# feos-org/feos-torch

Measured on AMD Instinct MI355X. Metric: pc_saft_pure_vapor_pressure_solves_per_sec, higher is better.
Workload: dtype f64 (fp32 pre-solve, fp64 finish)

## Files before the change

### feos_torch_amd/_lib.py

```python
import ctypes
import os

_HERE = os.path.dirname(os.path.abspath(__file__))
LIB_PATH = os.environ.get("PCS_HIP_LIB") or os.path.join(_HERE, "libpcsaft_hip.so")

_lib = None

_vp = ctypes.c_void_p
_i64 = ctypes.c_int64
_int = ctypes.c_int

SIGNATURES = {
    "pcs_abi_version": (_int, []),
    "pcs_last_error": (ctypes.c_char_p, []),
    "pcs_workspace_bytes": (_i64, [_i64]),
    "pcs_pure_vle": (_int, [_vp, _vp, _i64, _vp, _vp, _vp, _vp, _vp, _vp, _vp]),
    "pcs_pure_vapor_pressure": (_int, [_vp, _vp, _i64, _vp, _vp, _vp, _vp, _vp]),
    "pcs_compact_workspace_bytes": (_i64, [_i64]),
    "pcs_compact_plan": (_int, [_vp, _i64, _vp, _vp]),
    "pcs_compact_rows": (_int, [_vp, _i64, _vp, _vp, _int, _vp, _vp, _vp]),
    "pcs_expand_rows": (_int, [_vp, _i64, _vp, _vp, _vp, _int, _int, _int, _vp, _vp]),
    "pcs_pure_vle_fast": (_int, [_vp, _vp, _i64, _vp, _vp, _vp, _vp, _vp, _vp, _vp]),
    "pcs_pure_row_order": (_int, [_vp, _vp, _i64, _vp, _vp]),
    "pcs_pure_vle_fast_ordered": (_int, [_vp, _vp, _i64, _vp, _vp, _vp, _vp, _vp, _vp, _vp, _vp]),
    "pcs_pure_vle_fp64": (_int, [_vp, _vp, _i64, _vp, _vp, _vp, _vp, _vp, _vp, _vp]),
    "pcs_pure_vle_retry": (_int, [_vp, _vp, _i64, _vp, _vp, _vp, _vp, _vp, _vp, _vp]),
    "pcs_pure_liquid_density": (_int, [_vp, _vp, _vp, _i64, _vp, _vp, _vp, _vp]),
    "pcs_pure_derivatives": (_int, [_vp, _vp, _vp, _i64, _vp, _vp, _vp, _vp]),
    "pcs_pure_start_probe": (_int, [_vp, _vp, _i64, _vp, _vp]),
    "pcs_pure_jacobian": (_int, [_int, _vp, _vp, _vp, _vp, _i64, _vp, _vp]),
    "pcs_pure_jacobian_vjp": (_int, [_int, _vp, _vp, _vp, _vp, _vp, _i64, _vp, _vp, _vp, _vp]),
    "pcs_pure_critical_point": (_int, [_vp, _vp, _i64, _vp, _vp, _vp, _vp, _vp, _vp]),
    "pcs_pure_critical_point_vjp": (_int, [_vp, _vp, _vp, _i64, _vp, _vp, _vp, _vp, _vp]),
    "pcs_pure_boiling_temperature": (_int, [_vp, _vp, _vp, _i64, _vp, _vp, _vp, _vp, _vp]),
    "pcs_pure_enthalpy_of_vaporization": (_int, [_vp, _vp, _i64, _vp, _vp, _vp, _vp]),
    "pcs_pure_enthalpy_of_vaporization_vjp": (_int, [_vp, _vp, _vp, _i64, _vp, _vp, _vp, _vp]),
    "pcs_mix_workspace_bytes": (_i64, [_i64]),
    "pcs_mix_bubble_dew": (_int, [_int, _vp, _vp, _vp, _vp, _vp, _i64, _vp, _vp, _vp, _vp, _vp, _vp]),
    "pcs_mix_bubble_dew_temperature": (_int, [_int, _vp, _vp, _vp, _vp, _vp, _i64, _vp, _vp, _vp, _vp, _vp, _vp]),
    "pcs_mix_density": (_int, [_int, _vp, _vp, _vp, _vp, _vp, _i64, _vp, _vp, _vp, _vp, _vp, _vp]),
    "pcs_mix_henry": (_int, [_int, _vp, _vp, _vp, _i64, _vp, _vp, _vp, _vp, _vp, _vp]),
    "pcs_mix_jacobian": (_int, [_int, _vp, _vp, _vp, _vp, _i64, _vp, _vp, _vp]),
    "pcs_mix_point_jacobian": (_int, [_int, _vp, _vp, _vp, _vp, _i64, _vp, _vp, _vp, _vp]),
    "pcs_gc_table_doubles": (_i64, [_int]),
    "pcs_gc_bubble_dew": (_int, [_int, _vp, _int, _vp, _vp, _vp, _vp, _vp, _i64, _vp, _vp, _vp, _vp, _vp, _vp, _vp]),
    "pcs_gc_bubble_dew_temperature": (_int, [_int, _vp, _int, _vp, _vp, _vp, _vp, _vp, _i64, _vp, _vp, _vp, _vp, _vp, _vp]),
    "pcs_gc_density": (_int, [_int, _vp, _int, _vp, _vp, _vp, _vp, _vp, _i64, _vp, _vp, _vp, _vp, _vp, _vp]),
    "pcs_gc_pure_vle": (_int, [_int, _vp, _int, _vp, _vp, _vp, _i64, _vp, _vp, _vp, _vp, _vp, _vp, _vp]),
    "pcs_gc_derivatives": (_int, [_vp, _int, _vp, _vp, _vp, _vp, _i64, _vp, _vp, _vp, _vp, _vp]),
    "pcs_gc_jacobian": (_int, [_int, _vp, _int, _vp, _vp, _vp, _vp, _i64, _vp, _vp, _vp, _vp]),
    "pcs_gc_segment_gradient": (_int, [_int, _vp, _int, _vp, _vp, _vp, _vp, _i64, _vp, _vp, _vp, _vp]),
    "pcs_gc_point_jacobian": (_int, [_int, _vp, _int, _vp, _vp, _vp, _vp, _i64, _vp, _vp, _vp, _vp, _vp]),
    "pcs_gc_point_segment_gradient": (_int, [_int, _vp, _int, _vp, _vp, _vp, _vp, _i64, _vp, _vp, _vp, _vp, _vp]),
    "pcs_pure_derivatives_vjp": (_int, [_vp, _vp, _vp, _i64, _vp, _vp, _vp, _vp, _vp, _vp, _vp]),
    "pcs_mix_derivatives_vjp": (_int, [_vp, _vp, _vp, _vp, _i64, _vp, _vp, _vp, _vp, _vp, _vp, _vp]),
    "pcs_gc_derivatives_vjp": (_int, [_vp, _int, _vp, _vp, _vp, _vp, _i64, _vp, _vp, _vp, _vp, _vp, _vp, _vp, _vp, _vp]),
    "pcs_mixn_derivatives": (_int, [_vp, _vp, _vp, _int, _i64, _vp, _vp, _vp, _vp, _vp]),
    "pcs_mixn_derivatives_vjp": (_int, [_vp, _vp, _vp, _int, _i64, _vp, _vp, _vp, _vp, _vp, _vp]),
    "pcs_mix_derivatives": (_int, [_vp, _vp, _vp, _vp, _i64, _vp, _vp, _vp, _vp, _vp]),
    "pcs_mix_stability": (_int, [_vp, _vp, _vp, _vp, _i64, _vp, _vp, _vp, _vp]),
    "pcs_gc_stability": (_int, [_vp, _int, _vp, _vp, _vp, _vp, _i64, _vp, _vp, _vp, _vp, _vp]),
}


class PcsError(RuntimeError):
    pass


def lib():
    global _lib
    if _lib is None:
        if not os.path.exists(LIB_PATH):
            raise PcsError(
                f"{LIB_PATH} not found: build it with `python -c 'import __graft_entry__ as g; g.build()'` "
                "(hipcc --offload-arch=gfx950). There is no CPU fallback."
            )
        L = ctypes.CDLL(LIB_PATH)
        for name, (res, args) in SIGNATURES.items():
            fn = getattr(L, name)
            fn.restype = res
            fn.argtypes = args
        _lib = L
    return _lib


def check(rc, what):
    if rc != 0:
        msg = lib().pcs_last_error().decode("utf-8", "replace")
        raise PcsError(f"{what} failed (rc={rc}): {msg}")


def ptr(t):
    if t is None:
        return None
    return ctypes.c_void_p(t.data_ptr())


def current_stream_ptr(device):
    import torch

    return ctypes.c_void_p(torch.cuda.current_stream(device).cuda_stream)
```

### feos_torch_amd/csrc/pure_f32.hpp

```cpp
#pragma once
#include "pure_model.hpp"

namespace pcs {

constexpr float PCS_F32_TAYLOR_MAX = 1e-3f;
constexpr float PCS_F32_PREDICT_TOL_L = 5e-6f;
constexpr float PCS_F32_PREDICT_TOL_V = 5e-5f;
constexpr float PCS_F32_PREDICT_CMAX = 1e3f;
constexpr int PCS_F32_DENSE_LEVELS = 3;
constexpr float PCS_F32_LEAN_MAX = 0.5f;
constexpr float PCS_F32_SECANT_MIN = 3e-4f;
constexpr float PCS_F32_LIQ_TOL = 1e-1f;

struct F2 {
    float v, d1, d2;
};
PCS_DEV F2 f2(float v, float d1, float d2) { F2 r; r.v = v; r.d1 = d1; r.d2 = d2; return r; }
PCS_DEV F2 operator+(F2 a, F2 b) { return f2(a.v + b.v, a.d1 + b.d1, a.d2 + b.d2); }
PCS_DEV F2 operator-(F2 a, F2 b) { return f2(a.v - b.v, a.d1 - b.d1, a.d2 - b.d2); }
PCS_DEV F2 operator+(F2 a, float b) { return f2(a.v + b, a.d1, a.d2); }
PCS_DEV F2 operator-(float b, F2 a) { return f2(b - a.v, -a.d1, -a.d2); }
PCS_DEV F2 operator*(F2 a, float b) { return f2(a.v * b, a.d1 * b, a.d2 * b); }
PCS_DEV F2 operator*(F2 a, F2 b) {
    return f2(a.v * b.v, fmaf(a.d1, b.v, a.v * b.d1), fmaf(a.d2, b.v, fmaf(2.0f * a.d1, b.d1, a.v * b.d2)));
// ... 339 lines not shown
static_assert(start_close(START.SB[0], start_horner(B0, (double)PCS_F32_START_ETA)) && start_close(START.SB[1], start_horner(B1, (double)PCS_F32_START_ETA)) &&
              start_close(START.SB[2], start_horner(B2, (double)PCS_F32_START_ETA)), "eta-moments of B0..B2 against their Horner evaluation");
static_assert(start_close(start_log(6.0), 2.0 * start_log(2.0) + start_log(1.5)) && start_close(start_log(0.001) + start_log(1000.0), 0.0) &&
              start_close(start_log(2.718281828459045), 1.0), "compile-time logarithm");

PCS_DEV float start_rho_f32(const PureCoefF& c) { return PCS_F32_START_ETA / c.ceta; }

PCS_DEV EvalF pure_eval_start_f32(const PureCoefF& c) {
    constexpr StartConst K = START;
    const float rho = start_rho_f32(c);
    const float F = c.m * (float)K.HS.v - c.mm1 * (float)K.LG.v;
    const float Ft = c.m * (float)K.HS.t - c.mm1 * (float)K.LG.t;
    const float Ftt = c.m * (float)K.HS.tt - c.mm1 * (float)K.LG.tt;
    const float m1 = c.m1, m2 = c.m2;
    const float I1 = fmaf(m1, fmaf(m2, (float)K.SA[2].v, (float)K.SA[1].v), (float)K.SA[0].v);
    const float I1t = fmaf(m1, fmaf(m2, (float)K.SA[2].t, (float)K.SA[1].t), (float)K.SA[0].t);
    const float I1tt = fmaf(m1, fmaf(m2, (float)K.SA[2].tt, (float)K.SA[1].tt), (float)K.SA[0].tt);
    const float I2 = fmaf(m1, fmaf(m2, (float)K.SB[2].v, (float)K.SB[1].v), (float)K.SB[0].v);
    const float I2t = fmaf(m1, fmaf(m2, (float)K.SB[2].t, (float)K.SB[1].t), (float)K.SB[0].t);
    const float I2tt = fmaf(m1, fmaf(m2, (float)K.SB[2].tt, (float)K.SB[1].tt), (float)K.SB[0].tt);
    const float D = 1.0f + c.m * (float)K.A.v - c.mm1 * (float)K.B.v;
    const float Dt = c.m * (float)K.A.t - c.mm1 * (float)K.B.t;
    const float Dtt = c.m * (float)K.A.tt - c.mm1 * (float)K.B.tt;
    const float C = __builtin_amdgcn_rcpf(D), Csq = C * C;
    const float Ct = -Dt * Csq;
    const float Ctt = (2.0f * Dt * Dt * C - Dtt) * Csq;
    const float G = c.kd1 * I1 + c.kd2 * (C * I2);
    const float Gt = c.kd1 * I1t + c.kd2 * (Ct * I2 + C * I2t);
    const float Gtt = c.kd1 * I1tt + c.kd2 * (Ctt * I2 + 2.0f * Ct * I2t + C * I2tt);
    float a = rho * (F + rho * G);
    float at = rho * (F + Ft + rho * (2.0f * G + Gt));
    float att = rho * (2.0f * Ft + Ftt + rho * (2.0f * G + 4.0f * Gt + Gtt));
    if (c.polar || c.assoc) {
        if (c.polar) {
            float j1v = c.j1[0], j1t = 0.0f, j1tt = 0.0f, j2v = c.j2[0], j2t = 0.0f, j2tt = 0.0f;
#pragma unroll
            for (int i = 1; i < 5; i++) {
                j1v = fmaf(c.j1[i], K.pw.v[i], j1v);
                j1t = fmaf(c.j1[i], K.pw.t[i], j1t);
                if (i > 1) j1tt = fmaf(c.j1[i], K.pw.tt[i], j1tt);
            }
#pragma unroll
            for (int i = 1; i < 4; i++) {
                j2v = fmaf(c.j2[i], K.pw.v[i], j2v);
                j2t = fmaf(c.j2[i], K.pw.t[i], j2t);
                if (i > 1) j2tt = fmaf(c.j2[i], K.pw.tt[i], j2tt);
            }
            const F2 J1 = f2(j1v, j1t, j1tt);
            const F2 N = f2(j2v, j2t, j2tt) * rho;
            const F2 Q = (J1 * J1) * recipf(J1 - f2(N.v, N.d1 + N.v, N.d2 + 2.0f * N.d1));
            const float k = (rho * rho) * c.qm;
            a = fmaf(k, Q.v, a);
            at = fmaf(k, Q.d1 + 2.0f * Q.v, at);
            att = fmaf(k, Q.d2 + 4.0f * Q.d1 + 2.0f * Q.v, att);
        }
        if (c.assoc) {
            const float rd = rho * c.da;
            const float S = rd * (float)K.H.v, St = rd * (float)K.H.t, Stt = rd * (float)K.H.tt;
            float xa, xb;
            assoc_sites_f32(c, S, xa, xb);
            const float q = c.na * (f_log(xa) - 0.5f * xa + 0.5f) + c.nb * (f_log(xb) - 0.5f * xb + 0.5f);
            const float nn = c.na * c.nb;
            const float q1 = -nn * xa * xb;
            const float al = c.nb * xa * xa, be = c.na * xb * xb;
            const float rden = __builtin_amdgcn_rcpf(1.0f - al * be * S * S);
            const float xa1 = al * (be * S * xa - xb) * rden, xb1 = be * (al * S * xb - xa) * rden;
            const float q2 = -nn * (xa1 * xb + xa * xb1);
            a = fmaf(rho, q, a);
            at = fmaf(rho, q + q1 * St, at);
            att = fmaf(rho, q1 * (2.0f * St + Stt) + q2 * St * St, att);
        }
    }
    const float ir = c.ceta * (1.0f / PCS_F32_START_ETA);
    EvalF e;
    e.a = a;
    e.p = rho - a + at;
    e.dp = fmaf(att, ir, 1.0f);
    e.mu = at * ir;
    return e;
}

PCS_DEV bool finitef(float x) { return (__float_as_uint(x) & 0x7f800000u) != 0x7f800000u; }

struct LiquidRootF {
    float rl;
    bool ok, done, dense;
    int first;
};
template <bool AT_START>
PCS_DEV void liquid_root_step(const PureCoefF& f, float p_spec, float tol, float tol_dense, int it, const EvalF& e, LiquidRootF& s) {
    const float res = e.p - p_spec;
    const float eta = AT_START ? PCS_F32_START_ETA : s.rl * f.ceta;
    const int rung = AT_START ? 0 : eta < 0.575f ? 0 : eta < 0.655f ? 1 : eta < 0.735f ? 2 : PCS_F32_DENSE_LEVELS;
    if (it == s.first && rung < PCS_F32_DENSE_LEVELS && finitef(e.p) && !(res > 0.0f)) {
        s.dense = true;
        s.first = it + 1;
        float rn = (0.58f + 0.08f * (float)rung) / f.ceta;
        if (AT_START && e.dp > 0.0f) {
            const float r1 = s.rl - res * __builtin_amdgcn_rcpf(e.dp);
            const float eta1 = r1 * f.ceta;
            if (finitef(r1) && eta1 > PCS_F32_START_ETA && eta1 <= 0.74f) rn = r1;
        }
        s.rl = rn;
    } else if (!finitef(e.p) || !(e.dp > 0.0f) || (it == s.first && !(res > 0.0f))) {
        s.ok = false;
        s.done = true;
    } else {
        const float u = AT_START ? (float)START.u : __builtin_amdgcn_rcpf(1.0f - s.rl * f.ceta);
        float den = s.dense ? e.dp : e.dp - 4.0f * res * f.ceta * u;
        float step = res * __builtin_amdgcn_rcpf(den);
        if (!(den > 0.0f)) step = 2.0f * s.rl;
        float rn = s.rl - step;
        if (!(rn > 0.0f)) { s.ok = false; s.done = true; }
        else { s.done = fabsf(step) <= (s.dense ? tol_dense : tol) * s.rl; s.rl = rn; }
    }
}
PCS_DEV bool liquid_root_f32(const PureCoefF& f, float p_spec, float tol, float tol_dense, int cap, float& rl,
                             int& n_eval) {
    LiquidRootF s;
    s.ok = finitef(f.da) && finitef(f.kd2) && finitef(f.ceta) && f.ceta > 0.0f && finitef(p_spec);
    s.rl = start_rho_f32(f);
    s.done = !s.ok;
    s.dense = false;
    s.first = 0;
    if (cap > 0) {
        if (!s.done) {
            liquid_root_step<true>(f, p_spec, tol, tol_dense, 0, pure_eval_start_f32(f), s);
            n_eval++;
        }
        if (__ballot(!s.done) != 0ull) {
#pragma unroll 1
            for (int it = 1; it < cap; it++) {
                if (!s.done) {
                    liquid_root_step<false>(f, p_spec, tol, tol_dense, it, pure_eval_f32(f, s.rl), s);
                    n_eval++;
                }
                if (__ballot(!s.done) == 0ull) break;
            }
        }
    }
    rl = s.rl;
    return s.ok && s.done;
}

struct PreState {
    float rl, rv;
    EvalF l;
    float dpv;
    float sl_prev, sv_prev;
    float pv, dv_taken;
    float ev;
    float sec_prev, d_prev;
    bool lean_v;
    int it, n_liq, code;
    bool ok, done;
};

PCS_DEV void presolve_begin(const PureCoefF& f, PreState& s) {
    s.n_liq = 0; s.it = 0; s.code = 0;
    s.dpv = 1.0f; s.sl_prev = 1.0f; s.sv_prev = 1.0f;
    s.pv = 0.0f; s.dv_taken = 0.0f; s.ev = 0.0f; s.sec_prev = 0.0f; s.d_prev = 0.0f; s.lean_v = false;
    bool ok = liquid_root_f32(f, 0.0f, PCS_F32_LIQ_TOL, 1e-2f, 12, s.rl, s.n_liq);
    const float rl = s.rl;
    s.l = pure_eval_f32(f, rl);
    float rv = rl * f_exp(s.l.mu);
    {
        float B = (4.0f * f.m - 2.5f * f.mm1) * f.ceta + f.kd1 * f.ai[0] + f.kd2 * f.bi[0];
        if (f.polar) B += f.qm * f.j1[0];
        if (f.assoc) B -= f.na * f.nb * f.da;
        const float Lg = f_log(rv);
        float r = rv;
#pragma unroll
        for (int k = 0; k < 3; k++) {
            float den = fmaxf(1.0f + 2.0f * B * r, 0.3f);
            float fr = f_log(r) + 2.0f * B * r - Lg;
            r = r * fmaxf(1.0f - fr * __builtin_amdgcn_rcpf(den), 0.2f);
        }
        if (finitef(r) && r > 0.0f) rv = r;
    }
    s.code = !ok ? 1 : !finitef(rv) ? 6 : !(s.l.dp > 0.0f) ? 7 : !(rv < 0.5f * rl) ? 8 : !(rv > 1e-30f) ? 9 : 0;
    ok = ok && finitef(rv) && (s.l.dp > 0.0f) && (rv < 0.5f * rl) && (rv > 1e-30f);
    s.rv = rv;
    s.ok = ok;
    s.done = !ok;
}

PCS_DEV bool carry_slope(float p0, float p1, float drho, float s, float mu, float& dp, float& err, float& sec_prev, float& d_prev) {
    if (!(s * dp >= PCS_F32_SECANT_MIN * (1.0f + fabsf(mu)))) {
        d_prev = 0.0f;
        return true;
    }
    const float sec = (p1 - p0) * __builtin_amdgcn_rcpf(drho);
    const bool three = d_prev != 0.0f && fabsf(drho) <= 0.5f * fabsf(d_prev);
    const float cand = three ? fmaf(sec - sec_prev, drho * __builtin_amdgcn_rcpf(d_prev + drho), sec) : fmaf(2.0f, sec, -dp);
    if (!finitef(cand) || !(cand > 0.0f)) return false;
    const float rel = fabsf(cand * __builtin_amdgcn_rcpf(dp) - 1.0f);
    err = three ? 0.5f * rel * __builtin_amdgcn_sqrtf(err) : 0.25f * rel * rel;
    dp = cand;
    sec_prev = sec;
    d_prev = drho;
    return true;
}

PCS_DEV void presolve_coupled(const PureCoefF& f, PreState& s, int it_end) {
    float rl = s.rl, rv = s.rv;
    EvalF l = s.l;
    bool ok = s.ok, done = s.done;
    float dpv_last = s.dpv, dl_taken = 0.0f;
    float sl_prev = s.sl_prev, sv_prev = s.sv_prev;
    float pv_last = s.pv, dv_taken = s.dv_taken, ev = s.ev, sec_prev = s.sec_prev, d_prev = s.d_prev;
    bool lean_v = s.lean_v;
    int n_cpl = s.it;
    for (int it = 0; it < it_end; it++) {
        const bool act = !done && n_cpl < it_end;
        EvalF v;
        v.a = 0.0f; v.p = 0.0f; v.mu = 0.0f;
        bool full = act && !lean_v;
        const bool lean = act && lean_v;
        if (__ballot(lean) != 0ull) {
            if (lean) {
                const EvalF1 e = pure_eval1_f32(f, rv);
                v.a = e.a; v.p = e.p; v.mu = e.mu;
                full = !carry_slope(pv_last, e.p, dv_taken, sv_prev, e.mu, dpv_last, ev, sec_prev, d_prev);
            }
        }
        if (__ballot(full) != 0ull) {
            if (full) {
                v = pure_eval_f32(f, rv);
                dpv_last = v.dp;
                ev = 0.0f;
                d_prev = 0.0f;
            }
        }
        if (act) {
            v.dp = dpv_last;
            pv_last = v.p;
            float iv = __builtin_amdgcn_rcpf(rv), il = __builtin_amdgcn_rcpf(rl);
            float ps = -(v.a * iv - l.a * il + f_log(rv * il)) * __builtin_amdgcn_rcpf(iv - il);
            float dl = -(l.p - ps) * __builtin_amdgcn_rcpf(l.dp);
            float dv = -(v.p - ps) * __builtin_amdgcn_rcpf(v.dp);
            float rln = rl + dl, rvn = rv + dv;
            const bool log_step = rvn < 0.3f * rv;
            if (log_step) rvn = rv * f_exp(dv * iv);
            if (!finitef(rln) || !finitef(rvn) || !(v.dp > 0.0f) || !(l.dp > 0.0f) || !(rvn > 1e-30f) || !(rvn < 0.6f * rln)) {
                s.code = (!finitef(rln) || !finitef(rvn)) ? 10 : !(v.dp > 0.0f) ? 11 : !(l.dp > 0.0f) ? 12 : !(rvn > 1e-30f) ? 13 : 14;
                ok = false;
                done = true;
            } else {
                float sl = fabsf(dl) * il, sv = fabsf(dv) * iv;
                float pl = sl * sl * fminf(sl * __builtin_amdgcn_rcpf(sl_prev * sl_prev), PCS_F32_PREDICT_CMAX);
                float pv = sv * fmaf(sv, fminf(sv * __builtin_amdgcn_rcpf(sv_prev * sv_prev), PCS_F32_PREDICT_CMAX), ev);
                done = ((sl <= 2e-6f) && (sv <= 3e-5f)) || (n_cpl > 0 && sl < 1e-2f && sv < 1e-2f && pl <= PCS_F32_PREDICT_TOL_L && pv <= PCS_F32_PREDICT_TOL_V);
                sl_prev = sl; sv_prev = sv;
                dl_taken = rln - rl;
                dv_taken = rvn - rv;
                lean_v = !log_step && sv <= PCS_F32_LEAN_MAX;
                rl = rln;
                rv = rvn;
            }
            n_cpl++;
        }
        {
            const bool moved = act && !done;
            const bool reeval = moved && !(fabsf(dl_taken) <= PCS_F32_TAYLOR_MAX * rl);
            if (moved && !reeval) {
                const float a2 = (l.dp - 1.0f) * __builtin_amdgcn_rcpf(rl - dl_taken);
                l.a = fmaf(dl_taken, fmaf(0.5f * a2, dl_taken, l.mu), l.a);
                l.mu = fmaf(a2, dl_taken, l.mu);
                l.p = fmaf(l.dp, dl_taken, l.p);
            }
            if (__ballot(reeval) != 0ull) {
                if (reeval) l = pure_eval_f32(f, rl);
            }
        }
        if (__ballot(!done && n_cpl < it_end) == 0ull) break;
    }
    s.rl = rl; s.rv = rv; s.l = l; s.dpv = dpv_last; s.sl_prev = sl_prev; s.sv_prev = sv_prev;
    s.pv = pv_last; s.dv_taken = dv_taken; s.ev = ev; s.sec_prev = sec_prev; s.d_prev = d_prev; s.lean_v = lean_v;
    s.it = n_cpl; s.ok = ok; s.done = done;
}

PCS_DEV bool vle_presolve_f32(const PureCoefF& f, double& rl_out, double& rv_out, float& dpl_out, float& dpv_out,
                              int* diag = nullptr) {
    PreState s;
    presolve_begin(f, s);
    presolve_coupled(f, s, 8);
    rl_out = (double)s.rl;
    rv_out = (double)s.rv;
    dpl_out = s.l.dp;
    dpv_out = s.dpv;
    if (diag) *diag = s.n_liq | (s.it << 8) | (s.code << 16);
    return s.ok;
}

}
```

### feos_torch_amd/csrc/pure_kernels.hip

```cpp
#include "../../include/pcsaft_hip.h"
#include "abi_common.hpp"
#include "pure_vle_rows.hpp"
#include "pure_jacobian.hpp"

using namespace pcs_abi;

thread_local char pcs_abi::g_err[256] = "";

namespace {

constexpr int BLOCK = STAGE_BLOCK;
constexpr int ROW_PAD = STAGE_ROW_PAD;

__global__ __launch_bounds__(BLOCK, K1_WAVES_LITE) void k_pure_vle_rho(const double* __restrict__ params,
                                                    const double* __restrict__ temp, int64_t n,
                                                    double* __restrict__ p_sat, double* __restrict__ rho_eq,
                                                    double* __restrict__ rho_vl, uint8_t* __restrict__ status,
                                                    int32_t* __restrict__ iters, int32_t* __restrict__ retry) {
    pure_vle_rows<true, false, true>(params, temp, n, p_sat, rho_eq, rho_vl, status, iters, retry);
}

__global__ __launch_bounds__(BLOCK, K1_WAVES_LITE) void k_pure_vle_ordered(const double* __restrict__ params,
                                                    const double* __restrict__ temp, int64_t n,
                                                    double* __restrict__ p_sat, uint8_t* __restrict__ status,
                                                    int32_t* __restrict__ iters, int32_t* __restrict__ retry,
                                                    const int32_t* __restrict__ order) {
    pure_vle_rows<true, false, false, true>(params, temp, n, p_sat, nullptr, nullptr, status, iters, retry, order);
}

constexpr int ORDER_TILE = 16384;
constexpr int ORDER_TAU_BINS = 8;
constexpr int ORDER_BINS = K1_BINS * ORDER_TAU_BINS;
constexpr float ORDER_TAU_CAP = 2.0f;
static_assert(ORDER_TILE % BLOCK == 0 && ORDER_BINS <= BLOCK && ORDER_BINS <= 256, "one key byte per row, one lane per bin");
__device__ __forceinline__ float order_tau(const double* row, double T) {
    const float tau = (float)T / (1.28f * (float)row[2] * __powf((float)row[0], 0.45f));
    return fminf(fmaxf(tau, 0.0f), ORDER_TAU_CAP);
}
__global__ __launch_bounds__(BLOCK) void k_pure_row_order(const double* __restrict__ params, const double* __restrict__ temp,
                                                          int64_t n, int32_t* __restrict__ order_out) {
    __shared__ uint8_t keys[ORDER_TILE];
    __shared__ int bins[ORDER_BINS];
    __shared__ int range[2];
    const int t = threadIdx.x;
    const int64_t tile0 = (int64_t)blockIdx.x * ORDER_TILE;
    const int count = (int)min((int64_t)ORDER_TILE, n - tile0);
    if (t < ORDER_BINS) bins[t] = 0;
    if (t == 0) {
        range[0] = __float_as_int(ORDER_TAU_CAP);
        range[1] = 0;
    }
    __syncthreads();
    {
        float lo = ORDER_TAU_CAP, hi = 0.0f;
        for (int j = t; j < count; j += BLOCK) {
            const float tau = order_tau(params + 8 * (tile0 + j), temp[tile0 + j]);
            lo = fminf(lo, tau);
            hi = fmaxf(hi, tau);
        }
        atomicMin(&range[0], __float_as_int(lo));
        atomicMax(&range[1], __float_as_int(hi));
    }
    __syncthreads();
    const float tau_lo = __int_as_float(range[0]), width = __int_as_float(range[1]) - tau_lo;
    const float per_tau = width > 0.0f ? (float)ORDER_TAU_BINS / width : 0.0f;
    for (int j = t; j < count; j += BLOCK) {
        const double* row = params + 8 * (tile0 + j);
        const int bin = (int)fminf((order_tau(row, temp[tile0 + j]) - tau_lo) * per_tau, (float)(ORDER_TAU_BINS - 1));
        const int key = k1_bucket(row) * ORDER_TAU_BINS + max(bin, 0);
        keys[j] = (uint8_t)key;
        atomicAdd(&bins[key], 1);
    }
    __syncthreads();
    if (t == 0) {
        int acc = 0;
        for (int b = 0; b < ORDER_BINS; b++) {
            const int c = bins[b];
            bins[b] = acc;
            acc += c;
        }
    }
    __syncthreads();
    for (int j = t; j < count; j += BLOCK) order_out[tile0 + atomicAdd(&bins[keys[j]], 1)] = (int32_t)(tile0 + j);
}

constexpr int FALLBACK_GRID = 1024;
__global__ __launch_bounds__(64) void k_pure_vle_fallback(const double* __restrict__ params, const double* __restrict__ temp,
                                                          double* __restrict__ p_sat, double* __restrict__ rho_eq,
                                                          double* __restrict__ rho_vl,
                                                          uint8_t* __restrict__ status, int32_t* __restrict__ iters,
                                                          int32_t* __restrict__ retry, int64_t n) {
    const int count = (int)min((int64_t)max(retry[0], 0), n);
    for (int k = blockIdx.x * blockDim.x + threadIdx.x; k < count; k += gridDim.x * blockDim.x) {
        const uint32_t entry = (uint32_t)retry[1 + k];
        if (!(entry & 0x80000000u)) continue;
        const int64_t i = (int64_t)(entry & 0x7fffffffu);
        if (i >= n) continue;
        double par[8];
#pragma unroll
        for (int j = 0; j < 8; j++) par[j] = params[8 * i + j];
        const double T = temp[i];
        VleResult res;
        int st = rho_eq ? vle_fast<false>(par, T, res, 1e-8, TOL_STEP) : vle_fast<false>(par, T, res, TOL_L_P, TOL_V_P, rho_vl != nullptr);
        if (st == ST_OK) {
            if (p_sat) p_sat[i] = res.p_star * T * P_UNIT;
            if (rho_eq) rho_eq[i] = res.rho_l * (1.0 / RHO_UNIT);
            if (rho_vl) {
                rho_vl[2 * i] = res.rho_v;
                rho_vl[2 * i + 1] = res.rho_l;
            }
            if (iters) iters[i] = res.iters;
            status[i] = 0;
        } else {
            retry[1 + k] = (int32_t)i;
        }
    }
}

__global__ __launch_bounds__(BLOCK) void k_pure_derivatives(const double* __restrict__ params,
                                                            const double* __restrict__ temp,
                                                            const double* __restrict__ rho_in, int64_t n,
                                                            double* __restrict__ a, double* __restrict__ p,
                                                            double* __restrict__ dp) {
    const LaneRow row = stage_lane_row(params, n);
    const int64_t i = row.i, ii = row.ii;
    PureCoef<double> c;
    pure_coef<double>(c, row.par, temp[ii], false);
    Eval e = pure_eval(c, rho_in[ii]);
    if (!row.live) return;
    if (a) a[i] = e.a;
    if (p) p[i] = e.p;
    if (dp) dp[i] = e.dp;
}

__global__ __launch_bounds__(BLOCK) void k_pure_start_probe(const double* __restrict__ params, const double* __restrict__ temp,
                                                            int64_t n, float* __restrict__ out) {
    const int64_t i = (int64_t)blockIdx.x * BLOCK + threadIdx.x;
    if (i >= n) return;
    double par[8];
#pragma unroll
    for (int k = 0; k < 8; k++) par[k] = params[8 * i + k];
    PureCoefF f;
    pure_coef_f32(f, par, temp[i]);
    const EvalF g = pure_eval_f32(f, start_rho_f32(f));
    const EvalF s = pure_eval_start_f32(f);
    float* o = out + 8 * i;
    o[0] = g.a; o[1] = g.p; o[2] = g.dp; o[3] = g.mu;
    o[4] = s.a; o[5] = s.p; o[6] = s.dp; o[7] = s.mu;
}

constexpr int K4_WAVES = 2;
template <int WHICH>
__global__ __launch_bounds__(BLOCK, K4_WAVES) void k_pure_jacobian(const double* __restrict__ params,
                                                         const double* __restrict__ temp,
                                                         const double* __restrict__ pressure,
                                                         const double* __restrict__ rho_vl, int64_t n,
                                                         double* __restrict__ jac, const double* __restrict__ gout,
                                                         double* __restrict__ grad_params, double* __restrict__ grad_temp,
                                                         double* __restrict__ grad_press, int polish) {
    __shared__ double lds[BLOCK * ROW_PAD];
    const int64_t row0 = (int64_t)blockIdx.x * BLOCK;
    double par[8];
    constexpr bool BUCKET = WHICH == 1 || WHICH == 2;
    __shared__ int perm[BUCKET ? BLOCK : 1];
    __shared__ int bins[K1_BINS];
    const int t = threadIdx.x;
    if (BUCKET) block_order_reset<K1_BINS>(bins);
    stage_rows(params, n, row0, lds, par);
    int src = t;
    if (BUCKET) {
        block_order_sort<K1_BINS>(bins, perm, [=] { return k1_bucket(&lds[t * ROW_PAD]); });
        src = perm[t];
#pragma unroll
        for (int q = 0; q < 8; q++) par[q] = lds[src * ROW_PAD + q];
    }
    const int64_t i = row0 + src;
    const bool live = i < n;
    const int64_t ii = live ? i : n - 1;
    const double T = temp[ii];
    const double p_pa = (WHICH == 1) ? pressure[ii] : 0.0;
    const double rv = rho_vl[2 * ii], rl = rho_vl[2 * ii + 1];
    double g[10];
    pure_jacobian<WHICH>(par, T, p_pa, rv, rl, g, polish != 0);
    if (!live) return;
    if (jac) {
#pragma unroll
        for (int k = 0; k < 10; k++) jac[10 * i + k] = g[k];
    }
    if (gout) {
        const double w = gout[i];
        if (grad_params) {
            double2* dst = reinterpret_cast<double2*>(grad_params + 8 * i);
#pragma unroll
            for (int k = 0; k < 4; k++) dst[k] = make_double2(w * g[2 * k], w * g[2 * k + 1]);
        }
        if (grad_temp) grad_temp[i] = (WHICH == 3) ? 0.0 : w * g[8];
        if (grad_press) grad_press[i] = w * g[9];
    }
}

__global__ __launch_bounds__(BLOCK) void k_pure_derivatives_vjp(const double* __restrict__ params,
                                                                const double* __restrict__ temp,
                                                                const double* __restrict__ rho_in, int64_t n,
                                                                const double* __restrict__ g_a, const double* __restrict__ g_p,
                                                                const double* __restrict__ g_dp,
                                                                double* __restrict__ grad_params, double* __restrict__ grad_temp,
                                                                double* __restrict__ grad_rho) {
    const LaneRow row = stage_lane_row(params, n);
    const int64_t i = row.i, ii = row.ii;
    double g[VJP_DIRS];
    pure_derivatives_vjp(row.par, temp[ii], rho_in[ii], g_a ? g_a[ii] : 0.0, g_p ? g_p[ii] : 0.0, g_dp ? g_dp[ii] : 0.0, g);
    if (!row.live) return;
    if (grad_params) {
#pragma unroll
        for (int k = 0; k < 8; k++) grad_params[8 * i + k] = g[k];
    }
    if (grad_temp) grad_temp[i] = g[8];
    if (grad_rho) grad_rho[i] = g[9];
}

}

extern "C" {

int pcs_abi_version(void) { return 118; }

const char* pcs_last_error(void) { return g_err; }

int64_t pcs_workspace_bytes(int64_t n) { return (int64_t)sizeof(int32_t) * (n + 64); }

enum class VleKernel { LITE, LITE_POLISH, LITE_RHO, FP64, ORDERED };
enum class VleEntry { VLE, FP64, VAPOR_PRESSURE, ORDERED };

static VleKernel vle_main_kernel(VleEntry entry, bool rho_eq, bool rho_vl) {
    if (entry == VleEntry::ORDERED) return VleKernel::ORDERED;
    if (entry == VleEntry::FP64) return VleKernel::FP64;
    if (rho_eq) return VleKernel::LITE_POLISH;
    if (!rho_vl) return VleKernel::LITE;
    return entry == VleEntry::VAPOR_PRESSURE ? VleKernel::LITE_RHO : VleKernel::FP64;
}

enum : int { VLE_STAGE_FAST = 1, VLE_STAGE_RETRY = 2 };
static int pure_vle_stages(int stages, VleEntry entry, const double* params, const double* temp, int64_t n, double* p_sat,
                           double* rho_eq, double* rho_vl, uint8_t* status, int32_t* iters, void* workspace, void* stream,
                           const int32_t* order = nullptr) {
    if (int e = enter(n, params && temp && status && workspace, "pcs_pure_vle: null required pointer"); e != GO_ON) return e;
    int32_t* retry = static_cast<int32_t*>(workspace);
    hipStream_t s = as_stream(stream);
    if (stages & VLE_STAGE_FAST) {
        if (int ez = zero_ints(retry, 1, s)) return ez;
        const dim3 grid(grid_for(n, BLOCK)), block(BLOCK);
        const VleKernel main = vle_main_kernel(entry, rho_eq, rho_vl);
        switch (main) {
            case VleKernel::LITE: hipLaunchKernelGGL((k_pure_vle<true, false>), grid, block, 0, s, params, temp, n, p_sat, rho_eq, rho_vl, status, iters, retry); break;
            case VleKernel::LITE_POLISH: hipLaunchKernelGGL((k_pure_vle<true, true>), grid, block, 0, s, params, temp, n, p_sat, rho_eq, rho_vl, status, iters, retry); break;
            case VleKernel::LITE_RHO: hipLaunchKernelGGL(k_pure_vle_rho, grid, block, 0, s, params, temp, n, p_sat, rho_eq, rho_vl, status, iters, retry); break;
            case VleKernel::ORDERED: hipLaunchKernelGGL(k_pure_vle_ordered, grid, block, 0, s, params, temp, n, p_sat, status, iters, retry, order); break;
            case VleKernel::FP64:
                if (int ef = launch_pure_vle_full(params, temp, n, p_sat, rho_eq, rho_vl, status, iters, retry, s)) return ef;
        }
        hipLaunchKernelGGL(k_pure_vle_fallback, dim3(FALLBACK_GRID), dim3(64), 0, s, params, temp, p_sat, rho_eq, rho_vl, status,
                           iters, retry, n);
        if (int e = launched(main == VleKernel::ORDERED ? "k_pure_vle_ordered launch" : "k_pure_vle launch")) return e;
    }
    if (stages & VLE_STAGE_RETRY) return launch_pure_vle_retry(params, temp, p_sat, rho_eq, rho_vl, status, iters, retry, n, s);
    return 0;
}

int pcs_pure_vle(const double* params, const double* temp, int64_t n, double* p_sat, double* rho_eq,
                 double* rho_vl, uint8_t* status, int32_t* iters, void* workspace, void* stream) {
    return pure_vle_stages(VLE_STAGE_FAST | VLE_STAGE_RETRY, VleEntry::VLE, params, temp, n, p_sat, rho_eq, rho_vl, status, iters,
                           workspace, stream);
}

int pcs_pure_vle_fp64(const double* params, const double* temp, int64_t n, double* p_sat, double* rho_eq,
                      double* rho_vl, uint8_t* status, int32_t* iters, void* workspace, void* stream) {
    return pure_vle_stages(VLE_STAGE_FAST | VLE_STAGE_RETRY, VleEntry::FP64, params, temp, n, p_sat, rho_eq, rho_vl, status, iters,
                           workspace, stream);
}

int pcs_pure_vapor_pressure(const double* params, const double* temp, int64_t n, double* p_sat, double* rho_vl,
                            uint8_t* status, void* workspace, void* stream) {
    return pure_vle_stages(VLE_STAGE_FAST | VLE_STAGE_RETRY, VleEntry::VAPOR_PRESSURE, params, temp, n, p_sat, nullptr, rho_vl, status,
                           nullptr, workspace, stream);
}

int pcs_pure_vle_fast(const double* params, const double* temp, int64_t n, double* p_sat, double* rho_eq,
                      double* rho_vl, uint8_t* status, int32_t* iters, void* workspace, void* stream) {
    return pure_vle_stages(VLE_STAGE_FAST, VleEntry::VLE, params, temp, n, p_sat, rho_eq, rho_vl, status, iters, workspace, stream);
}

int pcs_pure_row_order(const double* params, const double* temp, int64_t n, int32_t* order_out, void* stream) {
    if (int e = enter(n, params && temp && order_out, "pcs_pure_row_order: null required pointer"); e != GO_ON) return e;
    hipLaunchKernelGGL(k_pure_row_order, dim3(grid_for(n, ORDER_TILE)), dim3(BLOCK), 0, as_stream(stream), params, temp, n, order_out);
    return launched("k_pure_row_order launch");
}

int pcs_pure_vle_fast_ordered(const double* params, const double* temp, int64_t n, double* p_sat, double* rho_eq, double* rho_vl,
                              uint8_t* status, int32_t* iters, void* workspace, const int32_t* order, void* stream) {
    if (int e = enter(n, params && temp && status && workspace && order, "pcs_pure_vle_fast_ordered: null required pointer"); e != GO_ON) return e;
    if (rho_eq || rho_vl) return fail_msg("pcs_pure_vle_fast_ordered", "pressure-only form: rho_eq and rho_vl must be null");
    return pure_vle_stages(VLE_STAGE_FAST, VleEntry::ORDERED, params, temp, n, p_sat, nullptr, nullptr, status, iters, workspace, stream,
                           order);
}

int pcs_pure_vle_retry(const double* params, const double* temp, int64_t n, double* p_sat, double* rho_eq,
                       double* rho_vl, uint8_t* status, int32_t* iters, void* workspace, void* stream) {
    return pure_vle_stages(VLE_STAGE_RETRY, VleEntry::VLE, params, temp, n, p_sat, rho_eq, rho_vl, status, iters, workspace, stream);
}

int pcs_pure_liquid_density(const double* params, const double* temp, const double* pressure, int64_t n,
                            double* rho_out, double* rho_root, uint8_t* status, void* stream) {
    if (int e = enter(n, params && temp && pressure && status, "pcs_pure_liquid_density: null required pointer"); e != GO_ON) return e;
    return launch_pure_liquid_density(params, temp, pressure, n, rho_out, rho_root, status, as_stream(stream));
}

int pcs_pure_derivatives(const double* params, const double* temp, const double* rho, int64_t n, double* a,
                         double* p, double* dp, void* stream) {
    if (int e = enter(n, params && temp && rho, "pcs_pure_derivatives: null required pointer"); e != GO_ON) return e;
    const unsigned grid = grid_for(n, BLOCK);
    hipLaunchKernelGGL(k_pure_derivatives, dim3(grid), dim3(BLOCK), 0, as_stream(stream), params, temp, rho, n, a, p,
                       dp);
    return launched("k_pure_derivatives launch");
}

int pcs_pure_start_probe(const double* params, const double* temp, int64_t n, float* out, void* stream) {
    if (int e = enter(n, params && temp && out, "pcs_pure_start_probe: null required pointer"); e != GO_ON) return e;
    const unsigned grid = grid_for(n, BLOCK);
    hipLaunchKernelGGL(k_pure_start_probe, dim3(grid), dim3(BLOCK), 0, as_stream(stream), params, temp, n, out);
    return launched("k_pure_start_probe launch");
}

int pcs_pure_derivatives_vjp(const double* params, const double* temp, const double* rho, int64_t n, const double* g_a,
                             const double* g_p, const double* g_dp, double* grad_params, double* grad_temp, double* grad_rho,
                             void* stream) {
    if (int e = enter(n, params && temp && rho, "pcs_pure_derivatives_vjp: null required pointer"); e != GO_ON) return e;
    const unsigned grid = grid_for(n, BLOCK);
    hipLaunchKernelGGL(k_pure_derivatives_vjp, dim3(grid), dim3(BLOCK), 0, as_stream(stream), params, temp, rho, n, g_a, g_p,
                       g_dp, grad_params, grad_temp, grad_rho);
    return launched("k_pure_derivatives_vjp launch");
}

static int launch_pure_jacobian(const char* entry, int which, const double* params, const double* temp, const double* pressure,
                                const double* rho_vl, int64_t n, double* jac, const double* gout, double* grad_params,
                                double* grad_temp, double* grad_pressure, hipStream_t s) {
    const int polish = (which & PCS_JAC_POLISH) ? 1 : 0;
    which &= ~PCS_JAC_POLISH;
    if (which == 1 && !pressure) return fail_msg(entry, "pressure required for liquid_density");
    if (int e = aligned16(entry, "grad_params", grad_params)) return e;
    const unsigned grid = grid_for(n, BLOCK);
    switch (which) {
        case 0: hipLaunchKernelGGL(k_pure_jacobian<0>, dim3(grid), dim3(BLOCK), 0, s, params, temp, pressure, rho_vl, n, jac, gout, grad_params, grad_temp, grad_pressure, polish); break;
        case 1: hipLaunchKernelGGL(k_pure_jacobian<1>, dim3(grid), dim3(BLOCK), 0, s, params, temp, pressure, rho_vl, n, jac, gout, grad_params, grad_temp, grad_pressure, polish); break;
        case 2: hipLaunchKernelGGL(k_pure_jacobian<2>, dim3(grid), dim3(BLOCK), 0, s, params, temp, pressure, rho_vl, n, jac, gout, grad_params, grad_temp, grad_pressure, polish); break;
        case 3: hipLaunchKernelGGL(k_pure_jacobian<3>, dim3(grid), dim3(BLOCK), 0, s, params, temp, pressure, rho_vl, n, jac, gout, grad_params, grad_temp, grad_pressure, polish); break;
        default: return fail_msg(entry, "which must be 0, 1, 2 or 3");
    }
    return launched("k_pure_jacobian launch");
}

int pcs_pure_jacobian(int which, const double* params, const double* temp, const double* pressure,
                      const double* rho_vl, int64_t n, double* jac, void* stream) {
    if (int e = enter(n, params && temp && rho_vl && jac, "pcs_pure_jacobian: null required pointer"); e != GO_ON) return e;
    return launch_pure_jacobian("pcs_pure_jacobian", which, params, temp, pressure, rho_vl, n, jac, nullptr, nullptr, nullptr, nullptr,
                                as_stream(stream));
}

int pcs_pure_jacobian_vjp(int which, const double* params, const double* temp, const double* pressure, const double* rho_vl,
                          const double* gout, int64_t n, double* grad_params, double* grad_temp, double* grad_pressure,
                          void* stream) {
    if (int e = enter(n, params && temp && rho_vl && gout, "pcs_pure_jacobian_vjp: null required pointer"); e != GO_ON) return e;
    return launch_pure_jacobian("pcs_pure_jacobian_vjp", which, params, temp, pressure, rho_vl, n, nullptr, gout, grad_params, grad_temp,
                                grad_pressure, as_stream(stream));
}

}
```

### include/pcsaft_hip.h

```cpp
#ifndef PCSAFT_HIP_H
#define PCSAFT_HIP_H

#include <stdint.h>

#ifdef __cplusplus
extern "C" {
#endif

int pcs_abi_version(void);

const char* pcs_last_error(void);

int64_t pcs_workspace_bytes(int64_t n);

int pcs_pure_vle(const double* params, const double* temp, int64_t n, double* p_sat, double* rho_eq,
                 double* rho_vl, uint8_t* status, int32_t* iters, void* workspace, void* stream);

int pcs_pure_vle_fast(const double* params, const double* temp, int64_t n, double* p_sat, double* rho_eq,
                      double* rho_vl, uint8_t* status, int32_t* iters, void* workspace, void* stream);
int pcs_pure_vle_retry(const double* params, const double* temp, int64_t n, double* p_sat, double* rho_eq,
                       double* rho_vl, uint8_t* status, int32_t* iters, void* workspace, void* stream);

int pcs_pure_row_order(const double* params, const double* temp, int64_t n, int32_t* order_out, void* stream);
int pcs_pure_vle_fast_ordered(const double* params, const double* temp, int64_t n, double* p_sat, double* rho_eq,
                              double* rho_vl, uint8_t* status, int32_t* iters, void* workspace, const int32_t* order,
                              void* stream);

int pcs_pure_vle_fp64(const double* params, const double* temp, int64_t n, double* p_sat, double* rho_eq,
                      double* rho_vl, uint8_t* status, int32_t* iters, void* workspace, void* stream);

int pcs_pure_vapor_pressure(const double* params, const double* temp, int64_t n, double* p_sat, double* rho_vl,
                            uint8_t* status, void* workspace, void* stream);

int pcs_pure_liquid_density(const double* params, const double* temp, const double* pressure, int64_t n,
                            double* rho_out, double* rho_root, uint8_t* status, void* stream);

int pcs_pure_derivatives(const double* params, const double* temp, const double* rho, int64_t n, double* a,
                         double* p, double* dp, void* stream);

int pcs_pure_start_probe(const double* params, const double* temp, int64_t n, float* out, void* stream);

#define PCS_JAC_POLISH 0x100
int pcs_pure_jacobian(int which, const double* params, const double* temp, const double* pressure,
                      const double* rho_vl, int64_t n, double* jac, void* stream);

int pcs_pure_jacobian_vjp(int which, const double* params, const double* temp, const double* pressure, const double* rho_vl,
                          const double* gout, int64_t n, double* grad_params, double* grad_temp, double* grad_pressure,
                          void* stream);

int pcs_pure_critical_point(const double* params, const double* t_init, int64_t n, double* tc, double* pc, double* rhoc,
                            uint8_t* status, int32_t* iters, void* stream);

int pcs_pure_critical_point_vjp(const double* params, const double* tc, const double* rhoc, int64_t n, const double* g_tc,
                                const double* g_pc, const double* g_rhoc, double* grad_params, void* stream);

int pcs_pure_boiling_temperature(const double* params, const double* pressure, const double* t_init, int64_t n, double* temp,
                                 double* rho_vl, uint8_t* status, int32_t* iters, void* stream);

int pcs_pure_enthalpy_of_vaporization(const double* params, const double* temp, int64_t n, double* dh, double* rho_vl,
                                      uint8_t* status, void* stream);

int pcs_pure_enthalpy_of_vaporization_vjp(const double* params, const double* temp, const double* rho_vl, int64_t n,
                                          const double* g_dh, double* g_params, double* g_temp, void* stream);

int64_t pcs_mix_workspace_bytes(int64_t n);
int pcs_mix_bubble_dew(int dew, const double* params, const double* kij, const double* temp, const double* z,
                       const double* p_init, int64_t n, double* p_out, double* rho4, uint8_t* status, int32_t* iters,
                       void* workspace, void* stream);

int pcs_mix_bubble_dew_temperature(int dew, const double* params, const double* kij, const double* p_spec, const double* z,
                                   const double* t_init, int64_t n, double* t_out, double* rho4, uint8_t* status,
                                   int32_t* iters, void* workspace, void* stream);

int pcs_mix_density(int phase, const double* params, const double* kij, const double* temp, const double* pressure,
                    const double* x, int64_t n, double* rho, double* dpdrho, uint8_t* status, int32_t* iters,
                    void* workspace, void* stream);

int pcs_mix_henry(int solute, const double* params, const double* kij, const double* temp, int64_t n, double* h,
                  double* rho_vl, double* p_sat, double* dlnh_drho, uint8_t* status, void* stream);

int pcs_mix_derivatives(const double* params, const double* kij, const double* temp, const double* rho, int64_t n,
                        double* a, double* p, double* mu, double* v, void* stream);

int pcs_mix_stability(const double* params, const double* kij, const double* temp, const double* rho, int64_t n,
                      double* tpd, double* rho_trial, uint8_t* status, void* stream);

int pcs_mixn_derivatives(const double* params, const double* temp, const double* rho, int ncomp, int64_t n, double* a, double* p,
                         double* mu, double* v, void* stream);

int pcs_mixn_derivatives_vjp(const double* params, const double* temp, const double* rho, int ncomp, int64_t n, const double* g_a,
                             const double* g_p, const double* g_mu, const double* g_v, double* grad, void* stream);

int pcs_mix_jacobian(int dew, const double* params, const double* kij, const double* temp, const double* rho4,
                     int64_t n, double* jac, void* workspace, void* stream);

int pcs_mix_point_jacobian(int dew, const double* params, const double* kij, const double* temp, const double* rho4,
                           int64_t n, double* jac_p, double* jac_y, void* workspace, void* stream);

int64_t pcs_gc_table_doubles(int S);
int pcs_gc_bubble_dew(int dew, const double* table, int S, const uint8_t* rows, const double* phi, const double* temp,
                      const double* z, const double* p_init, int64_t n, double* p_out, double* rho4, uint8_t* status,
                      int32_t* iters, const int32_t* order, void* workspace, void* stream);

int pcs_gc_bubble_dew_temperature(int dew, const double* table, int S, const uint8_t* rows, const double* phi,
                                  const double* p_spec, const double* z, const double* t_init, int64_t n, double* t_out,
                                  double* rho4, uint8_t* status, int32_t* iters, const int32_t* order, void* stream);

int pcs_gc_density(int phase, const double* table, int S, const uint8_t* rows, const double* phi, const double* temp,
                   const double* pressure, const double* x, int64_t n, double* rho, double* dpdrho, uint8_t* status,
// ... 53 lines not shown
```

Measured before the change: 16.79 billion.

## Order rows by fp32 presolve convergence signature instead of reduced temperature

Row ordering for the fast ordered VLE path now runs a full fp32 presolve per row, records convergence margins and flags, and buckets rows by these signatures within each k1 bucket. The goal is to group rows with similar iteration counts so wavefronts diverge less in the main solve. The bin prefix sum is also parallelised across lanes. The cost is an extra presolve pass before ordering, and whether this path runs depends on whether the benchmark uses row ordering, which is unknown.

```diff
diff --git a/feos_torch_amd/_lib.py b/feos_torch_amd/_lib.py
--- a/feos_torch_amd/_lib.py
+++ b/feos_torch_amd/_lib.py
@@ -22,6 +22,7 @@
     "pcs_expand_rows": (_int, [_vp, _i64, _vp, _vp, _vp, _int, _int, _int, _vp, _vp]),
     "pcs_pure_vle_fast": (_int, [_vp, _vp, _i64, _vp, _vp, _vp, _vp, _vp, _vp, _vp]),
     "pcs_pure_row_order": (_int, [_vp, _vp, _i64, _vp, _vp]),
+    "pcs_pure_order_key": (_int, [_vp, _vp, _i64, _vp, _vp, _vp]),
     "pcs_pure_vle_fast_ordered": (_int, [_vp, _vp, _i64, _vp, _vp, _vp, _vp, _vp, _vp, _vp, _vp]),
     "pcs_pure_vle_fp64": (_int, [_vp, _vp, _i64, _vp, _vp, _vp, _vp, _vp, _vp, _vp]),
     "pcs_pure_vle_retry": (_int, [_vp, _vp, _i64, _vp, _vp, _vp, _vp, _vp, _vp, _vp]),
diff --git a/feos_torch_amd/csrc/pure_f32.hpp b/feos_torch_amd/csrc/pure_f32.hpp
--- a/feos_torch_amd/csrc/pure_f32.hpp
+++ b/feos_torch_amd/csrc/pure_f32.hpp
@@ -445,12 +445,22 @@
 
 PCS_DEV bool finitef(float x) { return (__float_as_uint(x) & 0x7f800000u) != 0x7f800000u; }
 
+constexpr float PRE_MARGIN_OPEN = 1e30f;
+enum : int { PRE_SIG_REEVAL = 1, PRE_SIG_FULL_V = 2 };
+struct PreSignature {
+    int n_liq, n_cpl, code;
+    int flags;
+    float m_liq;
+    float m_l, m_v;
+};
+
 struct LiquidRootF {
     float rl;
     bool ok, done, dense;
     int first;
+    float m2;
 };
-template <bool AT_START>
+template <bool AT_START, bool SIG = false>
 PCS_DEV void liquid_root_step(const PureCoefF& f, float p_spec, float tol, float tol_dense, int it, const EvalF& e, LiquidRootF& s) {
     const float res = e.p - p_spec;
     const float eta = AT_START ? PCS_F32_START_ETA : s.rl * f.ceta;
@@ -475,12 +485,21 @@
         if (!(den > 0.0f)) step = 2.0f * s.rl;
         float rn = s.rl - step;
         if (!(rn > 0.0f)) { s.ok = false; s.done = true; }
-        else { s.done = fabsf(step) <= (s.dense ? tol_dense : tol) * s.rl; s.rl = rn; }
-    }
-}
+        else {
+            s.done = fabsf(step) <= (s.dense ? tol_dense : tol) * s.rl;
+            if constexpr (SIG) {
+                if (AT_START) s.m2 = s.done ? 0.0f : PRE_MARGIN_OPEN;
+                else if (it == 1) s.m2 = fabsf(step) * __builtin_amdgcn_rcpf((s.dense ? tol_dense : tol) * s.rl);
+            }
+            s.rl = rn;
+        }
+    }
+}
+template <bool SIG = false>
 PCS_DEV bool liquid_root_f32(const PureCoefF& f, float p_spec, float tol, float tol_dense, int cap, float& rl,
-                             int& n_eval) {
+                             int& n_eval, float* m2 = nullptr) {
     LiquidRootF s;
+    if constexpr (SIG) s.m2 = PRE_MARGIN_OPEN;
     s.ok = finitef(f.da) && finitef(f.kd2) && finitef(f.ceta) && f.ceta > 0.0f && finitef(p_spec);
     s.rl = start_rho_f32(f);
     s.done = !s.ok;
@@ -488,14 +507,14 @@
     s.first = 0;
     if (cap > 0) {
         if (!s.done) {
-            liquid_root_step<true>(f, p_spec, tol, tol_dense, 0, pure_eval_start_f32(f), s);
+            liquid_root_step<true, SIG>(f, p_spec, tol, tol_dense, 0, pure_eval_start_f32(f), s);
             n_eval++;
         }
         if (__ballot(!s.done) != 0ull) {
 #pragma unroll 1
             for (int it = 1; it < cap; it++) {
                 if (!s.done) {
-                    liquid_root_step<false>(f, p_spec, tol, tol_dense, it, pure_eval_f32(f, s.rl), s);
+                    liquid_root_step<false, SIG>(f, p_spec, tol, tol_dense, it, pure_eval_f32(f, s.rl), s);
                     n_eval++;
                 }
                 if (__ballot(!s.done) == 0ull) break;
@@ -503,6 +522,7 @@
         }
     }
     rl = s.rl;
+    if constexpr (SIG) *m2 = s.m2;
     return s.ok && s.done;
 }
 
@@ -517,13 +537,17 @@
     bool lean_v;
     int it, n_liq, code;
     bool ok, done;
+    float m_liq, m_l, m_v;
+    int flags;
 };
 
+template <bool SIG = false>
 PCS_DEV void presolve_begin(const PureCoefF& f, PreState& s) {
     s.n_liq = 0; s.it = 0; s.code = 0;
+    if constexpr (SIG) { s.m_liq = PRE_MARGIN_OPEN; s.m_l = 0.0f; s.m_v = 0.0f; s.flags = 0; }
     s.dpv = 1.0f; s.sl_prev = 1.0f; s.sv_prev = 1.0f;
     s.pv = 0.0f; s.dv_taken = 0.0f; s.ev = 0.0f; s.sec_prev = 0.0f; s.d_prev = 0.0f; s.lean_v = false;
-    bool ok = liquid_root_f32(f, 0.0f, PCS_F32_LIQ_TOL, 1e-2f, 12, s.rl, s.n_liq);
+    bool ok = liquid_root_f32<SIG>(f, 0.0f, PCS_F32_LIQ_TOL, 1e-2f, 12, s.rl, s.n_liq, &s.m_liq);
     const float rl = s.rl;
     s.l = pure_eval_f32(f, rl);
     float rv = rl * f_exp(s.l.mu);
@@ -565,6 +589,7 @@
     return true;
 }
 
+template <bool SIG = false>
 PCS_DEV void presolve_coupled(const PureCoefF& f, PreState& s, int it_end) {
     float rl = s.rl, rv = s.rv;
     EvalF l = s.l;
@@ -574,6 +599,9 @@
     float pv_last = s.pv, dv_taken = s.dv_taken, ev = s.ev, sec_prev = s.sec_prev, d_prev = s.d_prev;
     bool lean_v = s.lean_v;
     int n_cpl = s.it;
+    float m_l = 0.0f, m_v = 0.0f;
+    int flags = 0;
+    if constexpr (SIG) { m_l = s.m_l; m_v = s.m_v; flags = s.flags; }
     for (int it = 0; it < it_end; it++) {
         const bool act = !done && n_cpl < it_end;
         EvalF v;
@@ -590,6 +618,7 @@
         if (__ballot(full) != 0ull) {
             if (full) {
                 v = pure_eval_f32(f, rv);
+                if constexpr (SIG) { if (n_cpl >= 1) flags |= PRE_SIG_FULL_V; }
                 dpv_last = v.dp;
                 ev = 0.0f;
                 d_prev = 0.0f;
@@ -614,6 +643,10 @@
                 float pl = sl * sl * fminf(sl * __builtin_amdgcn_rcpf(sl_prev * sl_prev), PCS_F32_PREDICT_CMAX);
                 float pv = sv * fmaf(sv, fminf(sv * __builtin_amdgcn_rcpf(sv_prev * sv_prev), PCS_F32_PREDICT_CMAX), ev);
                 done = ((sl <= 2e-6f) && (sv <= 3e-5f)) || (n_cpl > 0 && sl < 1e-2f && sv < 1e-2f && pl <= PCS_F32_PREDICT_TOL_L && pv <= PCS_F32_PREDICT_TOL_V);
+                if constexpr (SIG) if (n_cpl == 1) {
+                    m_l = fmaxf(pl * (1.0f / PCS_F32_PREDICT_TOL_L), sl * 1e2f);
+                    m_v = fmaxf(pv * (1.0f / PCS_F32_PREDICT_TOL_V), sv * 1e2f);
+                }
                 sl_prev = sl; sv_prev = sv;
                 dl_taken = rln - rl;
                 dv_taken = rvn - rv;
@@ -633,7 +666,10 @@
                 l.p = fmaf(l.dp, dl_taken, l.p);
             }
             if (__ballot(reeval) != 0ull) {
-                if (reeval) l = pure_eval_f32(f, rl);
+                if (reeval) {
+                    l = pure_eval_f32(f, rl);
+                    if constexpr (SIG) { if (n_cpl >= 2) flags |= PRE_SIG_REEVAL; }
+                }
             }
         }
         if (__ballot(!done && n_cpl < it_end) == 0ull) break;
@@ -641,18 +677,20 @@
     s.rl = rl; s.rv = rv; s.l = l; s.dpv = dpv_last; s.sl_prev = sl_prev; s.sv_prev = sv_prev;
     s.pv = pv_last; s.dv_taken = dv_taken; s.ev = ev; s.sec_prev = sec_prev; s.d_prev = d_prev; s.lean_v = lean_v;
     s.it = n_cpl; s.ok = ok; s.done = done;
-}
-
+    if constexpr (SIG) { s.m_l = m_l; s.m_v = m_v; s.flags = flags; }
+}
+
+template <bool SIG = false>
 PCS_DEV bool vle_presolve_f32(const PureCoefF& f, double& rl_out, double& rv_out, float& dpl_out, float& dpv_out,
-                              int* diag = nullptr) {
+                              PreSignature* sig = nullptr) {
     PreState s;
-    presolve_begin(f, s);
-    presolve_coupled(f, s, 8);
+    presolve_begin<SIG>(f, s);
+    presolve_coupled<SIG>(f, s, 8);
     rl_out = (double)s.rl;
     rv_out = (double)s.rv;
     dpl_out = s.l.dp;
     dpv_out = s.dpv;
-    if (diag) *diag = s.n_liq | (s.it << 8) | (s.code << 16);
+    if constexpr (SIG) *sig = PreSignature{s.n_liq, s.it, s.code, s.flags, s.m_liq, s.m_l, s.m_v};
     return s.ok;
 }
 
diff --git a/feos_torch_amd/csrc/pure_kernels.hip b/feos_torch_amd/csrc/pure_kernels.hip
--- a/feos_torch_amd/csrc/pure_kernels.hip
+++ b/feos_torch_amd/csrc/pure_kernels.hip
@@ -29,57 +29,60 @@
 }
 
 constexpr int ORDER_TILE = 16384;
-constexpr int ORDER_TAU_BINS = 8;
-constexpr int ORDER_BINS = K1_BINS * ORDER_TAU_BINS;
-constexpr float ORDER_TAU_CAP = 2.0f;
+constexpr int ORDER_SUB = 64;
+constexpr int ORDER_BINS = K1_BINS * ORDER_SUB;
 static_assert(ORDER_TILE % BLOCK == 0 && ORDER_BINS <= BLOCK && ORDER_BINS <= 256, "one key byte per row, one lane per bin");
-__device__ __forceinline__ float order_tau(const double* row, double T) {
-    const float tau = (float)T / (1.28f * (float)row[2] * __powf((float)row[0], 0.45f));
-    return fminf(fmaxf(tau, 0.0f), ORDER_TAU_CAP);
-}
-__global__ __launch_bounds__(BLOCK) void k_pure_row_order(const double* __restrict__ params, const double* __restrict__ temp,
-                                                          int64_t n, int32_t* __restrict__ order_out) {
+constexpr int ORDER_MAJOR = 16, ORDER_MINOR = 4;
+static_assert(ORDER_MAJOR * ORDER_MINOR == ORDER_SUB, "sub-key = major * ORDER_MINOR + minor");
+__device__ __forceinline__ int order_exponent(float x) { return (int)((__float_as_uint(x) >> 23) & 0xffu) - 127; }
+__device__ __forceinline__ int order_subkey(const PreSignature& g) {
+    const float c = fminf(fmaxf(fmaxf(g.m_l, g.m_v), 0.03125f), 32.0f), q = fminf(fmaxf(g.m_liq, 0.03125f), 32.0f);
+    const int major = min(max(order_exponent(c * c) + 8, 0), ORDER_MAJOR - 1);
+    const int minor = min(max((order_exponent(q) + 4) >> 1, 0), ORDER_MINOR - 1);
+    return major * ORDER_MINOR + ((major & 1) ? ORDER_MINOR - 1 - minor : minor);
+}
+template <bool RAW>
+__global__ __launch_bounds__(BLOCK) void k_pure_order_key(const double* __restrict__ params, const double* __restrict__ temp,
+                                                          int64_t n, int32_t* __restrict__ key_out, int32_t* __restrict__ raw) {
+    const LaneRow row = stage_lane_row(params, n);
+    const double T = temp[row.ii];
+    PureCoefF f;
+    pure_coef_f32(f, row.par, T);
+    double rl, rv;
+    float dpl, dpv;
+    PreSignature sig;
+    const bool warm = vle_presolve_f32<true>(f, rl, rv, dpl, dpv, &sig);
+    if (!row.live) return;
+    bool usable = warm && is_finite_bits(T) && T > 0.0;
+#pragma unroll
+    for (int k = 0; k < 8; k++) usable = usable && is_finite_bits(row.par[k]) && (k > 2 || row.par[k] > 0.0);
+    key_out[row.i] = k1_bucket(row.par) * ORDER_SUB + (usable ? order_subkey(sig) : ORDER_SUB - 1);
+    if constexpr (RAW) {
+        int32_t* o = raw + 4 * row.i;
+        o[0] = (int32_t)((uint32_t)sig.n_liq | (uint32_t)sig.n_cpl << 8 | (uint32_t)sig.code << 16 | (uint32_t)sig.flags << 24 | (usable ? 0x80000000u : 0u));
+        o[1] = __float_as_int(sig.m_liq);
+        o[2] = __float_as_int(sig.m_l);
+        o[3] = __float_as_int(sig.m_v);
+    }
+}
+__global__ __launch_bounds__(BLOCK) void k_pure_row_order(int64_t n, int32_t* __restrict__ order_out) {
     __shared__ uint8_t keys[ORDER_TILE];
     __shared__ int bins[ORDER_BINS];
-    __shared__ int range[2];
     const int t = threadIdx.x;
     const int64_t tile0 = (int64_t)blockIdx.x * ORDER_TILE;
     const int count = (int)min((int64_t)ORDER_TILE, n - tile0);
     if (t < ORDER_BINS) bins[t] = 0;
-    if (t == 0) {
-        range[0] = __float_as_int(ORDER_TAU_CAP);
-        range[1] = 0;
-    }
     __syncthreads();
-    {
-        float lo = ORDER_TAU_CAP, hi = 0.0f;
-        for (int j = t; j < count; j += BLOCK) {
-            const float tau = order_tau(params + 8 * (tile0 + j), temp[tile0 + j]);
-            lo = fminf(lo, tau);
-            hi = fmaxf(hi, tau);
-        }
-        atomicMin(&range[0], __float_as_int(lo));
-        atomicMax(&range[1], __float_as_int(hi));
-    }
-    __syncthreads();
-    const float tau_lo = __int_as_float(range[0]), width = __int_as_float(range[1]) - tau_lo;
-    const float per_tau = width > 0.0f ? (float)ORDER_TAU_BINS / width : 0.0f;
     for (int j = t; j < count; j += BLOCK) {
-        const double* row = params + 8 * (tile0 + j);
-        const int bin = (int)fminf((order_tau(row, temp[tile0 + j]) - tau_lo) * per_tau, (float)(ORDER_TAU_BINS - 1));
-        const int key = k1_bucket(row) * ORDER_TAU_BINS + max(bin, 0);
+        const int key = min(max(order_out[tile0 + j], 0), ORDER_BINS - 1);
         keys[j] = (uint8_t)key;
         atomicAdd(&bins[key], 1);
     }
     __syncthreads();
-    if (t == 0) {
-        int acc = 0;
-        for (int b = 0; b < ORDER_BINS; b++) {
-            const int c = bins[b];
-            bins[b] = acc;
-            acc += c;
-        }
-    }
+    int first = 0;
+    for (int b = 0; b < t && b < ORDER_BINS; b++) first += bins[b];
+    __syncthreads();
+    if (t < ORDER_BINS) bins[t] = first;
     __syncthreads();
     for (int j = t; j < count; j += BLOCK) order_out[tile0 + atomicAdd(&bins[keys[j]], 1)] = (int32_t)(tile0 + j);
 }
@@ -223,7 +226,7 @@
 
 extern "C" {
 
-int pcs_abi_version(void) { return 118; }
+int pcs_abi_version(void) { return 119; }
 
 const char* pcs_last_error(void) { return g_err; }
 
@@ -292,8 +295,15 @@
 
 int pcs_pure_row_order(const double* params, const double* temp, int64_t n, int32_t* order_out, void* stream) {
     if (int e = enter(n, params && temp && order_out, "pcs_pure_row_order: null required pointer"); e != GO_ON) return e;
-    hipLaunchKernelGGL(k_pure_row_order, dim3(grid_for(n, ORDER_TILE)), dim3(BLOCK), 0, as_stream(stream), params, temp, n, order_out);
+    hipLaunchKernelGGL(k_pure_order_key<false>, dim3(grid_for(n, BLOCK)), dim3(BLOCK), 0, as_stream(stream), params, temp, n, order_out, nullptr);
+    hipLaunchKernelGGL(k_pure_row_order, dim3(grid_for(n, ORDER_TILE)), dim3(BLOCK), 0, as_stream(stream), n, order_out);
     return launched("k_pure_row_order launch");
+}
+
+int pcs_pure_order_key(const double* params, const double* temp, int64_t n, int32_t* key_out, int32_t* raw_out, void* stream) {
+    if (int e = enter(n, params && temp && key_out && raw_out, "pcs_pure_order_key: null required pointer"); e != GO_ON) return e;
+    hipLaunchKernelGGL(k_pure_order_key<true>, dim3(grid_for(n, BLOCK)), dim3(BLOCK), 0, as_stream(stream), params, temp, n, key_out, raw_out);
+    return launched("k_pure_order_key launch");
 }
 
 int pcs_pure_vle_fast_ordered(const double* params, const double* temp, int64_t n, double* p_sat, double* rho_eq, double* rho_vl,
diff --git a/include/pcsaft_hip.h b/include/pcsaft_hip.h
--- a/include/pcsaft_hip.h
+++ b/include/pcsaft_hip.h
@@ -25,6 +25,8 @@
 int pcs_pure_vle_fast_ordered(const double* params, const double* temp, int64_t n, double* p_sat, double* rho_eq,
                               double* rho_vl, uint8_t* status, int32_t* iters, void* workspace, const int32_t* order,
                               void* stream);
+
+int pcs_pure_order_key(const double* params, const double* temp, int64_t n, int32_t* key_out, int32_t* raw_out, void* stream);
 
 int pcs_pure_vle_fp64(const double* params, const double* temp, int64_t n, double* p_sat, double* rho_eq,
                       double* rho_vl, uint8_t* status, int32_t* iters, void* workspace, void* stream);
```

Result: faster. 17.80 billion (median of 6 runs) (+6.0%).
